# LinXueyuanStdio/LaTeX_OCR

Hardware: AMD Instinct MI355X
Metric: formula-images/sec training step (batch 64, 128x512) (higher is better)
Workload: dtype bf16

## Files before the change

### latex_ocr_amd/csrc/decoder_kernels.hip

```cpp
#include "decoder_kernels.h"
#include "api_util.h"
#include "drop.h"
#include <stdlib.h>

namespace {


LXO_DEV void load4(const float* p, float (&v)[4]) {
    f32x4 a = *reinterpret_cast<const f32x4*>(p);
    v[0] = a[0]; v[1] = a[1]; v[2] = a[2]; v[3] = a[3];
}
LXO_DEV void load4(const bf16_t* p, float (&v)[4]) {
    u32x2 a = *reinterpret_cast<const u32x2*>(p);
    v[0] = __uint_as_float(a[0] << 16); v[1] = __uint_as_float(a[0] & 0xffff0000u);
    v[2] = __uint_as_float(a[1] << 16); v[3] = __uint_as_float(a[1] & 0xffff0000u);
}
LXO_DEV void store4(float* p, const float (&v)[4]) { f32x4 a = {v[0], v[1], v[2], v[3]}; *reinterpret_cast<f32x4*>(p) = a; }
LXO_DEV void store4(bf16_t* p, const float (&v)[4]) { u32x2 a = {pack_bf2(v[0], v[1]), pack_bf2(v[2], v[3])}; *reinterpret_cast<u32x2*>(p) = a; }

LXO_DEV float slab_sum(const Slabs& sl, long long row, int col) {
    float v = 0.f;
    const float* q = sl.p + row * sl.ld + col;
    for (int s = 0; s < sl.n; ++s) v += q[(long long)s * sl.stride];
    return v;
// ... 809 lines not shown
#pragma unroll
            for (int j = 0; j < 4; ++j) rede[wave][k0 + j] = acc[kc][j] * b4[j];
        }
    }
    __syncthreads();
    for (int k = tid; k < E; k += 512) {
        float t = 0.f;
#pragma unroll
        for (int w = 0; w < ATT_W; ++w) t += rede[w][k];
        atomicAdd(&datth[(long long)v * E + k], t);
    }
}

typedef __amdgpu_buffer_rsrc_t ab_rsrc_t;
template <int ATT_U>
LXO_DEV void attb_load(u32x4 (&xi)[ATT_U], u32x2 (&xa)[ATT_U], float (&al)[ATT_U], ab_rsrc_t rim, ab_rsrc_t rai, ab_rsrc_t ral, int base, int n, int lane) {
#pragma unroll
    for (int u = 0; u < ATT_U; ++u) {
        const int r = max(min(base + ATT_W * u, n - 1), 0);
        xi[u] = __builtin_amdgcn_raw_buffer_load_b128(rim, lane * 16, r * 1024, 0);
        xa[u] = __builtin_amdgcn_raw_buffer_load_b64(rai, lane * 8, r * 512, 0);
        al[u] = __uint_as_float(__builtin_amdgcn_raw_buffer_load_b32(ral, 0, r * 4, 0));
    }
}
template <int ATT_U>
LXO_DEV void attb_block(const u32x4 (&xi)[ATT_U], const u32x2 (&xa)[ATT_U], const float (&al)[ATT_U], int base, int n, const float (&dc)[8],
                        const float (&ah)[4], float s, float (&acc)[4], float* de_row, int lane) {
    float pt[ATT_U];
#pragma unroll
    for (int u = 0; u < ATT_U; ++u) {
        float a = 0.f;
#pragma unroll
        for (int e = 0; e < 4; ++e) {
            a = fmaf(__uint_as_float(xi[u][e] << 16), dc[2 * e], a);
            a = fmaf(__uint_as_float(xi[u][e] & 0xffff0000u), dc[2 * e + 1], a);
        }
        pt[u] = a;
    }
#pragma unroll
    for (int o = 32; o > 0; o >>= 1) {
#pragma unroll
        for (int u = 0; u < ATT_U; ++u) pt[u] += __shfl_xor(pt[u], o);
    }
#pragma unroll
    for (int u = 0; u < ATT_U; ++u) {
        const int r = base + ATT_W * u;
        if (r >= n) continue;
        const float d = al[u] * (pt[u] - s);
        if (lane == 0) de_row[r] = d;
        const float x0 = __uint_as_float(xa[u][0] << 16), x1 = __uint_as_float(xa[u][0] & 0xffff0000u);
        const float x2 = __uint_as_float(xa[u][1] << 16), x3 = __uint_as_float(xa[u][1] & 0xffff0000u);
        const float t0 = tanh_ct<bf16_t>(x0 + ah[0]), t1 = tanh_ct<bf16_t>(x1 + ah[1]), t2 = tanh_ct<bf16_t>(x2 + ah[2]), t3 = tanh_ct<bf16_t>(x3 + ah[3]);
        acc[0] = fmaf(d, 1.f - t0 * t0, acc[0]); acc[1] = fmaf(d, 1.f - t1 * t1, acc[1]);
        acc[2] = fmaf(d, 1.f - t2 * t2, acc[2]); acc[3] = fmaf(d, 1.f - t3 * t3, acc[3]);
    }
}
template <int ATT_U>
__global__ __launch_bounds__(512) void attn_bwd_stream_kernel(const bf16_t* __restrict__ att_img, const bf16_t* __restrict__ img,
                                                             const float* __restrict__ att_h, const float* __restrict__ beta,
                                                             const float* __restrict__ alpha, const float* __restrict__ dctx, int lddc,
                                                             const float* __restrict__ ctx, int ldctx,
                                                             float* __restrict__ de, float* __restrict__ datth,
                                                             int R, int Rp, int rows_per, int rev) {
    constexpr int E = 256, C = 512;
    __shared__ float rede[ATT_W][E];
    const int ch = blockIdx.x, v = blockIdx.y;
    const int tid = threadIdx.x, lane = tid & 63, wave = __builtin_amdgcn_readfirstlane(tid >> 6);
    const int r0 = ch * rows_per;
    const int n = min(R, r0 + rows_per) - r0;
    if (n <= 0) return;
    const ab_rsrc_t rim = __builtin_amdgcn_make_buffer_rsrc(const_cast<bf16_t*>(img + ((long long)v * R + r0) * C), 0, n * C * 2, 0x00020000);
    const ab_rsrc_t rai = __builtin_amdgcn_make_buffer_rsrc(const_cast<bf16_t*>(att_img + ((long long)v * R + r0) * E), 0, n * E * 2, 0x00020000);
    const ab_rsrc_t ral = __builtin_amdgcn_make_buffer_rsrc(const_cast<float*>(alpha + (long long)v * Rp + r0), 0, n * 4, 0x00020000);
    const int nblk2 = ((n + ATT_W * ATT_U - 1) / (ATT_W * ATT_U) + 1) & ~1;
#define ABASE(i) (wave + ATT_W * ATT_U * (rev ? nblk2 - 1 - (i) : (i)))
    u32x4 xiA[ATT_U], xiB[ATT_U]; u32x2 xaA[ATT_U], xaB[ATT_U]; float alA[ATT_U], alB[ATT_U];
    attb_load<ATT_U>(xiA, xaA, alA, rim, rai, ral, ABASE(0), n, lane);
    attb_load<ATT_U>(xiB, xaB, alB, rim, rai, ral, ABASE(1), n, lane);
    const int c0 = lane * 8;
    const float* dp = dctx + (long long)v * lddc + c0;
    const float* cp = ctx + (long long)v * ldctx + c0;
    const f32x4 d0 = *reinterpret_cast<const f32x4*>(dp), d1 = *reinterpret_cast<const f32x4*>(dp + 4);
    const f32x4 x0 = *reinterpret_cast<const f32x4*>(cp), x1 = *reinterpret_cast<const f32x4*>(cp + 4);
    const f32x4 a4 = *reinterpret_cast<const f32x4*>(att_h + (long long)v * E + lane * 4);
    const f32x4 b4 = *reinterpret_cast<const f32x4*>(beta + lane * 4);
    float dc[8], ah[4], acc[4] = {0.f, 0.f, 0.f, 0.f};
#pragma unroll
    for (int e = 0; e < 4; ++e) { dc[e] = d0[e]; dc[4 + e] = d1[e]; ah[e] = a4[e]; }
    float s = 0.f;
#pragma unroll
    for (int e = 0; e < 4; ++e) s = fmaf(x0[e], dc[e], fmaf(x1[e], dc[4 + e], s));
    s = wave_sum(s);
    float* de_row = de + (long long)v * Rp + r0;
    for (int it = 0; it + 2 < nblk2; it += 2) {
        attb_block<ATT_U>(xiA, xaA, alA, ABASE(it), n, dc, ah, s, acc, de_row, lane);
        __builtin_amdgcn_sched_barrier(0);
        attb_load<ATT_U>(xiA, xaA, alA, rim, rai, ral, ABASE(it + 2), n, lane);
        __builtin_amdgcn_sched_barrier(0);
        attb_block<ATT_U>(xiB, xaB, alB, ABASE(it + 1), n, dc, ah, s, acc, de_row, lane);
        __builtin_amdgcn_sched_barrier(0);
        attb_load<ATT_U>(xiB, xaB, alB, rim, rai, ral, ABASE(it + 3), n, lane);
        __builtin_amdgcn_sched_barrier(0);
    }
    attb_block<ATT_U>(xiA, xaA, alA, ABASE(nblk2 - 2), n, dc, ah, s, acc, de_row, lane);
    attb_block<ATT_U>(xiB, xaB, alB, ABASE(nblk2 - 1), n, dc, ah, s, acc, de_row, lane);
#undef ABASE
#pragma unroll
    for (int j = 0; j < 4; ++j) rede[wave][lane * 4 + j] = acc[j] * b4[j];
    __syncthreads();
    if (tid < E) {
        float t = 0.f;
#pragma unroll
        for (int w = 0; w < ATT_W; ++w) t += rede[w][tid];
        atomicAdd(&datth[(long long)v * E + tid], t);
    }
}

__global__ __launch_bounds__(256) void att_exp_kernel(const bf16_t* __restrict__ x, bf16_t* __restrict__ out, long long n8) {
    for (long long i = (long long)blockIdx.x * 256 + threadIdx.x; i < n8; i += (long long)gridDim.x * 256) {
        float v[8];
        load8(x + i * 8, v);
#pragma unroll
        for (int e = 0; e < 8; ++e) v[e] = __builtin_amdgcn_exp2f(fminf(fmaxf(v[e] * 2.8853900817779268f, -60.f), 60.f));
        store8(out + i * 8, v);
    }
}

template <typename CT, int KCT>
__global__ __launch_bounds__(256) void datt_img_kernel(const CT* __restrict__ att_img, const float* __restrict__ att_h,
                                                      const float* __restrict__ beta, const float* __restrict__ de,
                                                      CT* __restrict__ dout, float* __restrict__ dbeta, float* __restrict__ dbeta_part,
                                                      int T, int B, int R, int Rp, int E) {
    __shared__ float redb[4][1024];
    const int b = blockIdx.y;
    const int tid = threadIdx.x, lane = tid & 63, wave = tid >> 6;
    const int KC = (E + 255) >> 8;
    float bt[KCT][4], db[KCT][4];
#pragma unroll
    for (int kc = 0; kc < KCT; ++kc) {
        const int k0 = kc * 256 + lane * 4;
#pragma unroll
        for (int j = 0; j < 4; ++j) { bt[kc][j] = (kc < KC && k0 + j < E) ? beta[k0 + j] : 0.f; db[kc][j] = 0.f; }
    }
    const int rbase = blockIdx.x * 16 + wave * 4;
    float x[4][KCT][4], acc[4][KCT][4];
#pragma unroll
    for (int rr = 0; rr < 4; ++rr)
#pragma unroll
        for (int kc = 0; kc < KCT; ++kc) {
            const int k0 = kc * 256 + lane * 4;
#pragma unroll
            for (int j = 0; j < 4; ++j) { x[rr][kc][j] = 0.f; acc[rr][kc][j] = 0.f; }
            if (rbase + rr < R && kc < KC && k0 < E) load4(att_img + ((long long)b * R + rbase + rr) * E + k0, x[rr][kc]);
            if constexpr (is_bf16<CT>::value) {
#pragma unroll
                for (int j = 0; j < 4; ++j) x[rr][kc][j] = __builtin_amdgcn_exp2f(fminf(fmaxf(x[rr][kc][j] * 2.8853900817779268f, -120.f), 120.f));
            }
        }
    float sumd = 0.f;
    if (rbase < R)
    for (int t0 = 0; t0 < T; t0 += 4) {
#pragma unroll
        for (int kc = 0; kc < KCT; ++kc) {
            const int k0 = kc * 256 + lane * 4;
            if (kc < KC && k0 < E) {
                float a[4][4], d[4][4];
#pragma unroll
                for (int tt = 0; tt < 4; ++tt) {
                    const int t = t0 + tt, tc = min(t, T - 1);
                    load4(att_h + ((long long)tc * B + b) * E + k0, a[tt]);
                    f32x4 dq = *reinterpret_cast<const f32x4*>(de + ((long long)tc * B + b) * Rp + rbase);
#pragma unroll
                    for (int rr = 0; rr < 4; ++rr) d[tt][rr] = (t < T && rbase + rr < R) ? dq[rr] : 0.f;
                    if constexpr (is_bf16<CT>::value) {
#pragma unroll
                        for (int j = 0; j < 4; ++j) a[tt][j] = __builtin_amdgcn_exp2f(fminf(fmaxf(a[tt][j] * 2.8853900817779268f, -120.f), 120.f));
                    }
                }
#pragma unroll
                for (int tt = 0; tt < 4; ++tt) {
                    if (d[tt][0] == 0.f && d[tt][1] == 0.f && d[tt][2] == 0.f && d[tt][3] == 0.f) continue;
#pragma unroll
                    for (int rr = 0; rr < 4; ++rr) {
                        const float dd = d[tt][rr];
                        if constexpr (is_bf16<CT>::value) {
                            const f32x2 d4 = {4.f * dd, 4.f * dd}, d2 = {dd, dd}, one = {1.f, 1.f};
                            sumd += dd;
#pragma unroll
                            for (int h = 0; h < 2; ++h) {
                                const f32x2 xs = {x[rr][kc][2 * h], x[rr][kc][2 * h + 1]}, as = {a[tt][2 * h], a[tt][2 * h + 1]};
                                const f32x2 w = __builtin_elementwise_fma(xs, as, one);
                                const f32x2 r = {__builtin_amdgcn_rcpf(w[0]), __builtin_amdgcn_rcpf(w[1])};
                                const f32x2 q = __builtin_elementwise_fma(-r, r, r);
                                f32x2 ac = {acc[rr][kc][2 * h], acc[rr][kc][2 * h + 1]}, dv = {db[kc][2 * h], db[kc][2 * h + 1]};
                                ac = __builtin_elementwise_fma(d4, q, ac);
                                dv = __builtin_elementwise_fma(d2, r, dv);
                                acc[rr][kc][2 * h] = ac[0]; acc[rr][kc][2 * h + 1] = ac[1];
                                db[kc][2 * h] = dv[0]; db[kc][2 * h + 1] = dv[1];
                            }
                        } else {
#pragma unroll
                            for (int j = 0; j < 4; ++j) {
                                const float tau = tanh_ct<CT>(x[rr][kc][j] + a[tt][j]);
                                acc[rr][kc][j] = fmaf(dd, 1.f - tau * tau, acc[rr][kc][j]);
                                db[kc][j] = fmaf(dd, tau, db[kc][j]);
                            }
                        }
                    }
                }
            }
        }
    }
#pragma unroll
    for (int rr = 0; rr < 4; ++rr)
#pragma unroll
        for (int kc = 0; kc < KCT; ++kc) {
            const int k0 = kc * 256 + lane * 4;
            if (rbase + rr < R && kc < KC && k0 < E) {
                float o[4];
#pragma unroll
                for (int j = 0; j < 4; ++j) o[j] = acc[rr][kc][j] * bt[kc][j];
                store4(dout + ((long long)b * R + rbase + rr) * E + k0, o);
            }
        }
#pragma unroll
    for (int kc = 0; kc < KCT; ++kc) {
        const int k0 = kc * 256 + lane * 4;
        if (kc < KC && k0 < E) {
#pragma unroll
            for (int j = 0; j < 4; ++j) redb[wave][k0 + j] = is_bf16<CT>::value ? sumd - 2.f * db[kc][j] : db[kc][j];
        }
    }
    __syncthreads();
    if (dbeta_part) {
        float* slot = dbeta_part + ((long long)blockIdx.y * gridDim.x + blockIdx.x) * E;
        for (int k = tid; k < E; k += 256) slot[k] = redb[0][k] + redb[1][k] + redb[2][k] + redb[3][k];
        return;
    }
    for (int k = tid; k < E; k += 256) atomicAdd(&dbeta[k], redb[0][k] + redb[1][k] + redb[2][k] + redb[3][k]);
}

__global__ __launch_bounds__(256) void add_mean_grad_kernel(float* __restrict__ dimg, const float* __restrict__ dmean, int B, int R, int C) {
    const long long total = (long long)B * R * C;
    const float inv = 1.0f / (float)R;
    for (long long i = (long long)blockIdx.x * 256 + threadIdx.x; i < total; i += (long long)gridDim.x * 256) {
        const int c = (int)(i % C);
        const int b = (int)(i / ((long long)R * C));
        dimg[i] += dmean[(long long)b * C + c] * inv;
    }
}

template <typename CT>
__global__ __launch_bounds__(256) void ce_loss_kernel(const float* __restrict__ logits, const int* __restrict__ formula,
                                                     const int* __restrict__ lengths, CT* __restrict__ dlogits,
                                                     float* __restrict__ loss_acc, float* __restrict__ loss_part, float inv_ntok, const float* __restrict__ ntok_dev,
                                                     const unsigned* __restrict__ chain_err, int B, int T, int V, int Vp) {
    __shared__ float red[8];
    if (chain_err && blockIdx.x == 0 && threadIdx.x == 0 && chain_err[0] != 0u) atomicAdd(&loss_acc[0], __uint_as_float(0x7fc00000u));
    if (ntok_dev) inv_ntok = 1.0f / ntok_dev[0];
    const int lane = threadIdx.x & 63, wave = threadIdx.x >> 6;
    float ce_sum = 0.f, n_sum = 0.f;
    for (int row = blockIdx.x * 4 + wave; row < T * B; row += gridDim.x * 4) {
        const int t = row / B, b = row - t * B;
        const float* lg = logits + (long long)row * Vp;
        CT* dl = dlogits + (long long)row * Vp;
        const bool valid = t < lengths[b];
        int tgt = formula[(long long)b * T + t];
        tgt = tgt < 0 ? 0 : (tgt >= V ? V - 1 : tgt);
        float m = -3.0e38f;
        for (int j = lane; j < V; j += 64) m = fmaxf(m, lg[j]);
        m = wave_max(m);
        float l = 0.f;
        for (int j = lane; j < V; j += 64) l += expf(lg[j] - m);
        l = wave_sum(l);
        const float lse = m + logf(l);
        const float scale = valid ? inv_ntok : 0.f;
        for (int j = lane; j < Vp; j += 64) {
            float g = 0.f;
            if (j < V) g = (expf(lg[j] - lse) - (j == tgt ? 1.f : 0.f)) * scale;
            dl[j] = from_f32<CT>(g);
        }
        if (valid) { ce_sum += lse - lg[tgt]; n_sum += 1.0f; }
    }
    if (lane == 0) { red[wave] = ce_sum; red[4 + wave] = n_sum; }
    __syncthreads();
    if (threadIdx.x == 0) {
        const float c = red[0] + red[1] + red[2] + red[3], n = red[4] + red[5] + red[6] + red[7];
        if (loss_part) { loss_part[2 * blockIdx.x] = c; loss_part[2 * blockIdx.x + 1] = n; }
        else if (n > 0.f) { atomicAdd(&loss_acc[0], c); atomicAdd(&loss_acc[1], n); }
    }
}

template <typename CT, int KV>
__global__ __launch_bounds__(256) void ce_loss_rows_kernel(const float* __restrict__ logits, const int* __restrict__ formula,
                                                          const int* __restrict__ lengths, CT* __restrict__ dlogits,
                                                          float* __restrict__ loss_acc, float* __restrict__ loss_part, float inv_ntok, const float* __restrict__ ntok_dev,
                                                          const unsigned* __restrict__ chain_err, int B, int T, int V, int Vp) {
    __shared__ float red[8];
    if (chain_err && blockIdx.x == 0 && threadIdx.x == 0 && chain_err[0] != 0u) atomicAdd(&loss_acc[0], __uint_as_float(0x7fc00000u));
    if (ntok_dev) inv_ntok = 1.0f / ntok_dev[0];
    const int lane = threadIdx.x & 63, wave = threadIdx.x >> 6;
    float ce_sum = 0.f, n_sum = 0.f;
    for (int row = blockIdx.x * 4 + wave; row < T * B; row += gridDim.x * 4) {
        const int t = row / B, b = row - t * B;
        const float* lg = logits + (long long)row * Vp;
        CT* dl = dlogits + (long long)row * Vp;
        const bool valid = t < lengths[b];
        int tgt = formula[(long long)b * T + t];
        tgt = tgt < 0 ? 0 : (tgt >= V ? V - 1 : tgt);
        const float xt = lg[tgt];
        float x[KV];
#pragma unroll
        for (int q = 0; q < KV / 4; ++q) {
            const int j0 = 4 * (lane + 64 * q);
            const f32x4 v = *reinterpret_cast<const f32x4*>(lg + (j0 < Vp ? j0 : 0));
#pragma unroll
            for (int e = 0; e < 4; ++e) x[4 * q + e] = (j0 + e < V) ? v[e] : -3.0e38f;
        }
        float m = x[0];
#pragma unroll
        for (int e = 1; e < KV; ++e) m = fmaxf(m, x[e]);
        m = wave_max(m);
        float l = 0.f;
#pragma unroll
        for (int e = 0; e < KV; ++e) l += is_bf16<CT>::value ? __expf(x[e] - m) : expf(x[e] - m);
        l = wave_sum(l);
        const float lse = m + logf(l);
        const float scale = valid ? inv_ntok : 0.f;
#pragma unroll
        for (int q = 0; q < KV / 4; ++q) {
            const int j0 = 4 * (lane + 64 * q);
            if (j0 >= Vp) continue;
            float g[4];
#pragma unroll
            for (int e = 0; e < 4; ++e) {
                const int j = j0 + e;
                const float pr = is_bf16<CT>::value ? __expf(x[4 * q + e] - lse) : expf(x[4 * q + e] - lse);
                g[e] = j < V ? (pr - (j == tgt ? 1.f : 0.f)) * scale : 0.f;
            }
            if constexpr (is_bf16<CT>::value) { const u32x2 pk = {pack_bf2(g[0], g[1]), pack_bf2(g[2], g[3])}; *reinterpret_cast<u32x2*>(dl + j0) = pk; }
            else { const f32x4 gv = {g[0], g[1], g[2], g[3]}; *reinterpret_cast<f32x4*>(dl + j0) = gv; }
        }
        if (valid) { ce_sum += lse - xt; n_sum += 1.0f; }
    }
    if (lane == 0) { red[wave] = ce_sum; red[4 + wave] = n_sum; }
    __syncthreads();
    if (threadIdx.x == 0) {
        const float c = red[0] + red[1] + red[2] + red[3], n = red[4] + red[5] + red[6] + red[7];
        if (loss_part) { loss_part[2 * blockIdx.x] = c; loss_part[2 * blockIdx.x + 1] = n; }
        else if (n > 0.f) { atomicAdd(&loss_acc[0], c); atomicAdd(&loss_acc[1], n); }
    }
}

__global__ __launch_bounds__(256) void colsum_kernel(const float* __restrict__ a, int lda, float* __restrict__ out, int M, int N, int rows_per_block) {
    const int n = blockIdx.x * 256 + threadIdx.x;
    const int m0 = blockIdx.y * rows_per_block, m1 = min(M, m0 + rows_per_block);
    if (n >= N) return;
    float s = 0.f;
    for (int m = m0; m < m1; ++m) s += a[(long long)m * lda + n];
    atomicAdd(&out[n], s);
}

__global__ __launch_bounds__(256) void colsum4_kernel(const float* __restrict__ a, int lda, float* __restrict__ out, int M, int N, int rows_per_block) {
    __shared__ f32x4 red[4][64];
    const int cq = threadIdx.x & 63, ry = threadIdx.x >> 6;
    const int n = (blockIdx.x * 64 + cq) * 4;
    const int m0 = blockIdx.y * rows_per_block, m1 = min(M, m0 + rows_per_block);
    const int nl = n < N ? n : 0;
    f32x4 s = {0.f, 0.f, 0.f, 0.f};
    for (int mb = m0 + ry; mb < m1; mb += 32) {
        f32x4 v[8];
#pragma unroll
        for (int u = 0; u < 8; ++u) { const int m = min(mb + 4 * u, m1 - 1); v[u] = *reinterpret_cast<const f32x4*>(a + (long long)m * lda + nl); }
#pragma unroll
        for (int u = 0; u < 8; ++u) if (mb + 4 * u < m1) s += v[u];
    }
    red[ry][cq] = s;
    __syncthreads();
    if (ry == 0 && n < N) {
        const f32x4 t = red[0][cq] + red[1][cq] + red[2][cq] + red[3][cq];
#pragma unroll
        for (int e = 0; e < 4; ++e) atomicAdd(&out[n + e], t[e]);
    }
}


template <typename AT>
__global__ __launch_bounds__(256) void colsum_part_kernel(const AT* __restrict__ a, long long lda, float* __restrict__ part, long long M, int N, int rows_per) {
    const int n = blockIdx.x * 256 + threadIdx.x;
    const long long m0 = (long long)blockIdx.y * rows_per, m1 = m0 + rows_per < M ? m0 + rows_per : M;
    if (n >= N) return;
    float s = 0.f;
// ... 722 lines not shown
    if (C % 64) return -2;
    if (dt == LXO_BF16) LAUNCH((rowmean_kernel<bf16_t>), dim3(C / 64, B), (const bf16_t*)img, mean, R, C);
    else LAUNCH((rowmean_kernel<float>), dim3(C / 64, B), (const float*)img, mean, R, C);
    DONE;
}
int lxo_k_embed_gather(int dt, const float* table, const float* start, const int* formula, void* out, int B, int T, int D, int Dp, int V, hipStream_t st) {
    const int g = grid1((long long)T * B * Dp);
    if (dt == LXO_BF16) LAUNCH((embed_gather_kernel<bf16_t>), g, table, start, formula, (bf16_t*)out, B, T, D, Dp, V);
    else LAUNCH((embed_gather_kernel<float>), g, table, start, formula, (float*)out, B, T, D, Dp, V);
    DONE;
}
int lxo_k_embed_rows(int dt, const float* table, const float* start, const int* ids, void* out, int n, int D, int Dp, int V, hipStream_t st) {
    const int g = grid1((long long)n * Dp);
    if (dt == LXO_BF16) LAUNCH((embed_rows_kernel<bf16_t>), g, table, start, ids, (bf16_t*)out, n, D, Dp, V);
    else LAUNCH((embed_rows_kernel<float>), g, table, start, ids, (float*)out, n, D, Dp, V);
    DONE;
}
int lxo_k_embed_table(int dt, const float* table, const float* start, void* out, int V, int D, int Dp, hipStream_t st) {
    const int g = grid1((long long)(V + 1) * Dp);
    if (dt == LXO_BF16) LAUNCH((embed_table_kernel<bf16_t>), g, table, start, (bf16_t*)out, V, D, Dp);
    else LAUNCH((embed_table_kernel<float>), g, table, start, (float*)out, V, D, Dp);
    DONE;
}
int lxo_k_lstm_fwd(const float* z, Slabs zs, const float* c_prev, float* gates, float* c_out, float* h_out, float* ht_out, int ldh, Drop dr, int B, int U, hipStream_t st) {
    LAUNCH(lstm_fwd_kernel, grid1((long long)B * U), z, zs, c_prev, gates, c_out, h_out, ht_out, ldh, dr, B, U);
    DONE;
}
int lxo_k_lstm_bwd(const float* gates, const float* c_prev, const float* c_cur, Slabs s1, Slabs s3, Slabs s4, int off4,
                   float* dcc, float* dz, Drop dr, int carry_rows, int B, int U, hipStream_t st) {
    LAUNCH(lstm_bwd_kernel, grid1((long long)B * U), gates, c_prev, c_cur, s1, s3, s4, off4, dcc, dz, dr, carry_rows, B, U);
    DONE;
}
int lxo_k_tanh_bwd(const float* a, int lda, Slabs carry, const float* o, int ldo, float* g, int ldg, void* gb, int ldgb, Drop dr, int carry_rows, int rows, int cols, hipStream_t st) {
    LAUNCH(tanh_bwd_kernel, grid1((long long)rows * cols / 4), a, lda, carry, o, ldo, g, ldg, (bf16_t*)gb, ldgb, dr, carry_rows, rows, cols);
    DONE;
}
__global__ __launch_bounds__(256) static void slab_reduce_kernel(Slabs sl, float* __restrict__ o, int ldo, int rows, int cols) {
    const int total = rows * (cols >> 2);
    for (int i = blockIdx.x * 256 + threadIdx.x; i < total; i += gridDim.x * 256) {
        const int r = i / (cols >> 2), c = (i - r * (cols >> 2)) << 2;
        *reinterpret_cast<f32x4*>(o + (long long)r * ldo + c) = slab_sum4(sl, r, c);
    }
}
int lxo_k_slab_reduce(Slabs sl, float* o, int ldo, int rows, int cols, hipStream_t st) {
    LAUNCH(slab_reduce_kernel, grid1((long long)rows * cols / 4), sl, o, ldo, rows, cols);
    DONE;
}
int lxo_k_tanh_finalize(Slabs sl, float* o, int ldo, Drop dr, int rows, int cols, hipStream_t st) {
    LAUNCH(tanh_finalize_kernel, grid1((long long)rows * cols / 4), sl, o, ldo, dr, rows, cols);
    DONE;
}
static int att_u(int rows_per) {
    static int forced = -1;
    if (forced < 0) { const char* e = getenv("LXO_ATT_U"); forced = e ? atoi(e) : 0; }
    if (forced == 7 || forced == 8) return forced;
    return (rows_per + 55) / 56 <= (rows_per + 63) / 64 ? 7 : 8;
}
int lxo_k_attn_fwd(int dt, const void* att_img, const void* img, const float* att_h, Slabs ahs, float* att_h_out, const float* beta, float* alpha, float* part,
                   float* ctx, int ldctx, void* ctxb, int ldcb, int nv, int R, int Rp, int E, int C, int beam, int nch, int rev, hipStream_t st, const void* att_exp) {
    if (E > 1024 || C > 512 || nch < 1 || nch > 32) return -2;
    const int rows_per = cdiv(R, nch);
    dim3 grid(nch, nv);
    static int split = -1;
    if (split < 0) { const char* e = getenv("LXO_ATT_SPLIT"); split = (e && e[0] == '1') ? 1 : 0; }
    const int epl = dt == LXO_BF16 ? 8 : 4;
    if (split && ahs.n == 0 && att_h && R <= 1024 && C % 64 == 0 && E % epl == 0 && E <= 64 * epl && ((E / epl) & (E / epl - 1)) == 0) {
        if (dt == LXO_BF16) {
            hipLaunchKernelGGL((attn_scores_kernel<bf16_t, 8>), grid, dim3(512), 0, st, (const bf16_t*)att_img, att_h, beta, part, R, Rp, E, beam, rows_per);
            hipLaunchKernelGGL((attn_ctx_kernel<bf16_t, 8>), dim3(C / 64, nv), dim3(512), 0, st, (const bf16_t*)img, part, alpha, ctx, ldctx, (bf16_t*)ctxb, ldcb, R, Rp, C, beam);
        } else {
            hipLaunchKernelGGL((attn_scores_kernel<float, 8>), grid, dim3(512), 0, st, (const float*)att_img, att_h, beta, part, R, Rp, E, beam, rows_per);
            hipLaunchKernelGGL((attn_ctx_kernel<float, 8>), dim3(C / 64, nv), dim3(512), 0, st, (const float*)img, part, alpha, ctx, ldctx, (bf16_t*)ctxb, ldcb, R, Rp, C, beam);
        }
        DONE;
    }
    static int beam_shared = -1;
    if (beam_shared < 0) { const char* e = getenv("LXO_ATT_BEAM_SHARED"); beam_shared = (e && e[0] == '0') ? 0 : 1; }
    if (beam_shared && (beam == 2 || beam == 3 || beam == 5 || (beam == 1 && att_exp && dt == LXO_BF16)) && ahs.n == 0 && att_h && E <= 256 && C <= 512 && nv % beam == 0) {
        const int nimg = nv / beam;
        int nb = cdiv(512, nimg);
        if (nb > 16) nb = 16;
        const int by_rows = R / 32 > 0 ? R / 32 : 1;
        if (nb > by_rows) nb = by_rows;
        const int need = cdiv(R, 1024);
        if (nb < need) nb = need;
        const int rpb = cdiv(R, nb);
        const dim3 gb(nb, nimg);
#define ABM(CT_, U_, NB_, X_, OCC_, AI_) hipLaunchKernelGGL((attn_fwd_part_beam_kernel<CT_, U_, NB_, X_, OCC_>), gb, dim3(512), 0, st, (const CT_*)(AI_), (const CT_*)img, att_h, beta, alpha, part, R, Rp, E, C, nb, rpb, rev)
        if (dt == LXO_BF16 && att_exp) { if (beam == 1) ABM(bf16_t, 4, 1, true, 4, att_exp); else if (beam == 2) ABM(bf16_t, 4, 2, true, 4, att_exp); else if (beam == 3) ABM(bf16_t, 4, 3, true, 4, att_exp); else ABM(bf16_t, 2, 5, true, 4, att_exp); }
        else if (dt == LXO_BF16) { if (beam == 2) ABM(bf16_t, 4, 2, false, 2, att_img); else if (beam == 3) ABM(bf16_t, 4, 3, false, 2, att_img); else ABM(bf16_t, 4, 5, false, 2, att_img); }
        else { if (beam == 2) ABM(float, 4, 2, false, 2, att_img); else if (beam == 3) ABM(float, 4, 3, false, 2, att_img); else ABM(float, 4, 5, false, 2, att_img); }
#undef ABM
        hipLaunchKernelGGL(attn_fwd_combine_kernel, dim3(4, nv), dim3(256), 0, st, part, alpha, ctx, ldctx, (bf16_t*)ctxb, ldcb, R, Rp, C, nb, rpb);
        DONE;
    }
#define AF_ARGS att_h, ahs, att_h_out, beta, alpha, part, R, Rp, E, C, beam, nch, rows_per, rev
    if (dt == LXO_BF16) {
        if (E <= 256) { if (att_u(rows_per) == 8) hipLaunchKernelGGL((attn_fwd_part_kernel<bf16_t, 1, 8>), grid, dim3(512), 0, st, (const bf16_t*)att_img, (const bf16_t*)img, AF_ARGS); else hipLaunchKernelGGL((attn_fwd_part_kernel<bf16_t, 1, 7>), grid, dim3(512), 0, st, (const bf16_t*)att_img, (const bf16_t*)img, AF_ARGS); }
        else { if (att_u(rows_per) == 8) hipLaunchKernelGGL((attn_fwd_part_kernel<bf16_t, 4, 8>), grid, dim3(512), 0, st, (const bf16_t*)att_img, (const bf16_t*)img, AF_ARGS); else hipLaunchKernelGGL((attn_fwd_part_kernel<bf16_t, 4, 7>), grid, dim3(512), 0, st, (const bf16_t*)att_img, (const bf16_t*)img, AF_ARGS); }
    } else {
        if (E <= 256) { if (att_u(rows_per) == 8) hipLaunchKernelGGL((attn_fwd_part_kernel<float, 1, 8>), grid, dim3(512), 0, st, (const float*)att_img, (const float*)img, AF_ARGS); else hipLaunchKernelGGL((attn_fwd_part_kernel<float, 1, 7>), grid, dim3(512), 0, st, (const float*)att_img, (const float*)img, AF_ARGS); }
        else { if (att_u(rows_per) == 8) hipLaunchKernelGGL((attn_fwd_part_kernel<float, 4, 8>), grid, dim3(512), 0, st, (const float*)att_img, (const float*)img, AF_ARGS); else hipLaunchKernelGGL((attn_fwd_part_kernel<float, 4, 7>), grid, dim3(512), 0, st, (const float*)att_img, (const float*)img, AF_ARGS); }
    }
#undef AF_ARGS
    hipLaunchKernelGGL(attn_fwd_combine_kernel, dim3(4, nv), dim3(256), 0, st, part, alpha, ctx, ldctx, (bf16_t*)ctxb, ldcb, R, Rp, C, nch, rows_per);
    DONE;
}
int lxo_k_att_exp(const void* att_img, void* att_exp, long long n, hipStream_t st) {
    if (n % 8) return -2;
    LAUNCH(att_exp_kernel, grid1(n / 8, 256, 4096), (const bf16_t*)att_img, (bf16_t*)att_exp, n / 8);
    DONE;
}
int lxo_k_attn_bwd(int dt, const void* att_img, const void* att_exp, const void* img, const float* att_h, const float* beta, const float* alpha,
                   Slabs dcs, int dcoff, float* dctx_out, int lddc, const float* ctx, int ldctx, float* de, float* datth,
                   int nv, int R, int Rp, int E, int C, int nch, int rev, hipStream_t st) {
    if (E > 1024 || C > 512 || nch < 1 || nch > 32) return -2;
    const int rows_per = cdiv(R, nch);
    dim3 grid(nch, nv);
    static int stream2 = -1;
    if (stream2 < 0) { const char* e = getenv("LXO_ATT_BWD2"); stream2 = (e && e[0] == '1') ? 1 : 0; }
    if (stream2 && dt == LXO_BF16 && E == 256 && C == 512 && dcs.n == 1 && lddc % 4 == 0 && ldctx % 4 == 0 && (long long)rows_per * 1024 < (1LL << 31)) {
        const float* dctx = dcs.p + dcoff;
        if (dctx_out) return -2;
        hipLaunchKernelGGL((attn_bwd_stream_kernel<4>), grid, dim3(512), 0, st, (const bf16_t*)att_img, (const bf16_t*)img, att_h, beta, alpha, dctx, dcs.ld,
                           ctx, ldctx, de, datth, R, Rp, rows_per, rev);
        DONE;
    }
#define AB_ARGS att_h, beta, alpha, dcs, dcoff, dctx_out, lddc, ctx, ldctx, de, datth, R, Rp, E, C, rows_per, rev
    if (dt == LXO_BF16 && att_exp && E <= 256) {
        if (att_u(rows_per) == 8) hipLaunchKernelGGL((attn_bwd_part_kernel<bf16_t, 1, 8, true>), grid, dim3(512), 0, st, (const bf16_t*)att_exp, (const bf16_t*)img, AB_ARGS);
        else hipLaunchKernelGGL((attn_bwd_part_kernel<bf16_t, 1, 7, true>), grid, dim3(512), 0, st, (const bf16_t*)att_exp, (const bf16_t*)img, AB_ARGS);
    } else if (dt == LXO_BF16) {
        if (E <= 256) { if (att_u(rows_per) == 8) hipLaunchKernelGGL((attn_bwd_part_kernel<bf16_t, 1, 8>), grid, dim3(512), 0, st, (const bf16_t*)att_img, (const bf16_t*)img, AB_ARGS); else hipLaunchKernelGGL((attn_bwd_part_kernel<bf16_t, 1, 7>), grid, dim3(512), 0, st, (const bf16_t*)att_img, (const bf16_t*)img, AB_ARGS); }
        else { if (att_u(rows_per) == 8) hipLaunchKernelGGL((attn_bwd_part_kernel<bf16_t, 4, 8>), grid, dim3(512), 0, st, (const bf16_t*)att_img, (const bf16_t*)img, AB_ARGS); else hipLaunchKernelGGL((attn_bwd_part_kernel<bf16_t, 4, 7>), grid, dim3(512), 0, st, (const bf16_t*)att_img, (const bf16_t*)img, AB_ARGS); }
    } else {
        if (E <= 256) { if (att_u(rows_per) == 8) hipLaunchKernelGGL((attn_bwd_part_kernel<float, 1, 8>), grid, dim3(512), 0, st, (const float*)att_img, (const float*)img, AB_ARGS); else hipLaunchKernelGGL((attn_bwd_part_kernel<float, 1, 7>), grid, dim3(512), 0, st, (const float*)att_img, (const float*)img, AB_ARGS); }
        else { if (att_u(rows_per) == 8) hipLaunchKernelGGL((attn_bwd_part_kernel<float, 4, 8>), grid, dim3(512), 0, st, (const float*)att_img, (const float*)img, AB_ARGS); else hipLaunchKernelGGL((attn_bwd_part_kernel<float, 4, 7>), grid, dim3(512), 0, st, (const float*)att_img, (const float*)img, AB_ARGS); }
    }
#undef AB_ARGS
    DONE;
}
int lxo_k_det_reduce(const float* part, int nslot, long long stride, int N, float* out, hipStream_t st) {
    if (nslot <= 0 || N <= 0) return 0;
    hipLaunchKernelGGL(det_reduce_kernel, dim3(cdiv(N, 16)), dim3(256), 0, st, part, nslot, stride, N, out);
    DONE;
}
int lxo_k_datt_img(int dt, const void* att_img, const float* att_h, const float* beta, const float* de, void* dout, float* dbeta,
                   int T, int B, int R, int Rp, int E, DetScratch det, hipStream_t st) {
    dim3 grid(cdiv(R, 16), B);
    if (E > 1024) return -2;
    float* part = nullptr;
    if (det.p) { if ((size_t)grid.x * grid.y * E > det.floats) return -6; part = det.p; }
    if (dt == LXO_BF16) {
        if (E <= 256) hipLaunchKernelGGL((datt_img_kernel<bf16_t, 1>), grid, dim3(256), 0, st, (const bf16_t*)att_img, att_h, beta, de, (bf16_t*)dout, dbeta, part, T, B, R, Rp, E);
        else hipLaunchKernelGGL((datt_img_kernel<bf16_t, 4>), grid, dim3(256), 0, st, (const bf16_t*)att_img, att_h, beta, de, (bf16_t*)dout, dbeta, part, T, B, R, Rp, E);
    } else {
        if (E <= 256) hipLaunchKernelGGL((datt_img_kernel<float, 1>), grid, dim3(256), 0, st, (const float*)att_img, att_h, beta, de, (float*)dout, dbeta, part, T, B, R, Rp, E);
        else hipLaunchKernelGGL((datt_img_kernel<float, 4>), grid, dim3(256), 0, st, (const float*)att_img, att_h, beta, de, (float*)dout, dbeta, part, T, B, R, Rp, E);
    }
    if (part) return lxo_k_det_reduce(part, (int)(grid.x * grid.y), E, E, dbeta, st);
    DONE;
}
int lxo_k_add_mean_grad(float* dimg, const float* dmean, int B, int R, int C, hipStream_t st) {
    LAUNCH(add_mean_grad_kernel, grid1((long long)B * R * C), dimg, dmean, B, R, C);
    DONE;
}
int lxo_k_ce_loss(int dt, const float* logits, const int* formula, const int* lengths, void* dlogits, float* loss_acc, float inv_ntok,
                  const float* ntok_dev, const unsigned* chain_err, int B, int T, int V, int Vp, DetScratch det, hipStream_t st) {
    int g = cdiv(T * B, 4);
    float* part = (det.p && det.floats >= 1024) ? det.p : nullptr;
    if (Vp % 4 == 0 && Vp <= 1024 && (((uintptr_t)logits | (uintptr_t)dlogits) & 15) == 0) {
        if (g > (part ? 512 : 2048)) g = part ? 512 : 2048;
#define CE_ROWS(CT_, KV_) LAUNCH((ce_loss_rows_kernel<CT_, KV_>), g, logits, formula, lengths, (CT_*)dlogits, loss_acc, part, inv_ntok, ntok_dev, chain_err, B, T, V, Vp)
        if (dt == LXO_BF16) { if (Vp <= 256) CE_ROWS(bf16_t, 4); else if (Vp <= 512) CE_ROWS(bf16_t, 8); else CE_ROWS(bf16_t, 16); }
        else { if (Vp <= 256) CE_ROWS(float, 4); else if (Vp <= 512) CE_ROWS(float, 8); else CE_ROWS(float, 16); }
#undef CE_ROWS
        if (part) return lxo_k_det_reduce(part, g, 2, 2, loss_acc, st);
        DONE;
    }
    if (g > 512) g = 512;
    if (dt == LXO_BF16) LAUNCH((ce_loss_kernel<bf16_t>), g, logits, formula, lengths, (bf16_t*)dlogits, loss_acc, part, inv_ntok, ntok_dev, chain_err, B, T, V, Vp);
    else LAUNCH((ce_loss_kernel<float>), g, logits, formula, lengths, (float*)dlogits, loss_acc, part, inv_ntok, ntok_dev, chain_err, B, T, V, Vp);
    if (part) return lxo_k_det_reduce(part, g, 2, 2, loss_acc, st);
    DONE;
}
int lxo_k_score(int dt, const float* logits, const int* formula, const int* lengths, float* logp_out, int* top1_out, float* seq_out,
                const unsigned* chain_err, int B, int T, int V, int Vp, hipStream_t st) {
    int g = cdiv(T * B, 4);
    if (Vp % 4 == 0 && Vp <= 1024 && ((uintptr_t)logits & 15) == 0) {
        if (g > 2048) g = 2048;
#define SC_ROWS(BF_, KV_) LAUNCH((score_rows_kernel<BF_, KV_>), g, logits, formula, lengths, logp_out, top1_out, chain_err, B, T, V, Vp)
        if (dt == LXO_BF16) { if (Vp <= 256) SC_ROWS(true, 4); else if (Vp <= 512) SC_ROWS(true, 8); else SC_ROWS(true, 16); }
        else { if (Vp <= 256) SC_ROWS(false, 4); else if (Vp <= 512) SC_ROWS(false, 8); else SC_ROWS(false, 16); }
#undef SC_ROWS
    } else {
        LAUNCH(score_kernel, g > 512 ? 512 : g, logits, formula, lengths, logp_out, top1_out, chain_err, B, T, V, Vp);
    }
    if (seq_out) LAUNCH(score_seq_kernel, cdiv(B, 256), logp_out, lengths, seq_out, chain_err, B, T);
    DONE;
}
int lxo_k_colsum_det(const void* a, int bf16, long long lda, float* out, long long M, int N, DetScratch det, hipStream_t st) {
    if (!det.p) return -6;
    if (M <= 0 || N <= 0) return 0;
    long long maxslots = (long long)(det.floats / (size_t)N);
    if (maxslots < 1) return -6;
    if (maxslots > 1024) maxslots = 1024;
    long long rows_per = (M + maxslots - 1) / maxslots;
    if (rows_per < 64) rows_per = 64;
    const int nrb = (int)((M + rows_per - 1) / rows_per);
    if (bf16) hipLaunchKernelGGL((colsum_part_kernel<bf16_t>), dim3(cdiv(N, 256), nrb), dim3(256), 0, st, (const bf16_t*)a, lda, det.p, M, N, (int)rows_per);
    else hipLaunchKernelGGL((colsum_part_kernel<float>), dim3(cdiv(N, 256), nrb), dim3(256), 0, st, (const float*)a, lda, det.p, M, N, (int)rows_per);
    return lxo_k_det_reduce(det.p, nrb, N, N, out, st);
}
int lxo_k_colsum(const float* a, long long lda, float* out, long long M, int N, DetScratch det, hipStream_t st) {
    if (det.p) return lxo_k_colsum_det(a, 0, lda, out, M, N, det, st);
    const int rpb = 64;
    if (N % 4 == 0 && lda % 4 == 0 && ((uintptr_t)a & 15) == 0 && M > 0)
        hipLaunchKernelGGL(colsum4_kernel, dim3(cdiv(N, 256), cdiv((int)M, rpb)), dim3(256), 0, st, a, (int)lda, out, (int)M, N, rpb);
    else
    hipLaunchKernelGGL(colsum_kernel, dim3(cdiv(N, 256), cdiv((int)M, rpb)), dim3(256), 0, st, a, (int)lda, out, (int)M, N, rpb);
    DONE;
}
int lxo_k_embed_scatter(const float* demb, const int* formula, float* dtable, float* dstart, int B, int T, int D, int V, int det, hipStream_t st) {
    if (D <= 256) { hipLaunchKernelGGL(embed_scatter_rows_kernel, dim3(V + 1, det ? 1 : 16), dim3(256), 0, st, demb, formula, dtable, dstart, B, T, D, V, det); DONE; }
    if (det) return -2;
    LAUNCH(embed_scatter_kernel, grid1((long long)T * B * D), demb, formula, dtable, dstart, B, T, D, V);
    DONE;
}
int lxo_k_init_bwd(const float* dcc, Slabs dxh, const float* c0, const float* rec0, int ldr, float* dpre, int B, int U, int O, hipStream_t st) {
    LAUNCH(init_bwd_kernel, grid1((long long)B * (2 * U + O)), dcc, dxh, c0, rec0, ldr, dpre, B, U, O);
    DONE;
}
#define DEC_VARIANT(KERNEL, grid, block, ...)                                                                         \
    do {                                                                                                               \
        if (prefix && allow) hipLaunchKernelGGL((KERNEL<true, true>), dim3(grid), dim3(block), 0, st, __VA_ARGS__);    \
        else if (prefix) hipLaunchKernelGGL((KERNEL<true, false>), dim3(grid), dim3(block), 0, st, __VA_ARGS__);       \
        else if (allow) hipLaunchKernelGGL((KERNEL<false, true>), dim3(grid), dim3(block), 0, st, __VA_ARGS__);        \
        else hipLaunchKernelGGL((KERNEL<false, false>), dim3(grid), dim3(block), 0, st, __VA_ARGS__);                  \
    } while (0)
int lxo_k_argmax(const float* logits, int Vp, int V, int n, int id_end, int* ids_step, int* ids_out, int max_steps, int step,
                 int* finished, int* n_unfinished, hipStream_t st, float* logp_out, const DecPrefix* prefix, const DecAllow* allow) {
    const DecPrefix pf = prefix ? *prefix : DecPrefix{};
    const DecAllow al = allow ? *allow : DecAllow{};
    DEC_VARIANT(argmax_kernel, cdiv(n, 4), 256, logits, Vp, V, n, id_end, ids_step, ids_out, max_steps, step, finished, n_unfinished, logp_out, pf, al);
    DONE;
}
int lxo_k_beam_step(float* logits, int Vp, int V, int nimg, int k, int id_end, int time, float div_gamma, float div_prob, int div_seed,
                    float* scratch, float* logp, int* finished,
                    int* ids_step, int* parents_step, int* ids_out, int* par_out, int max_steps, int* n_unfinished, hipStream_t st,
                    float* scores_out, const DecPrefix* prefix, const DecAllow* allow) {
    if (k > 16 || k > V) return -2;
    DivPen dp = {0.f, 0u, (unsigned)div_seed, scratch};
    if (div_gamma > 0.f && div_gamma != 1.f && div_prob > 0.f) {
        dp.log_gamma = logf(div_gamma);
        dp.thr = div_prob >= 1.f ? 16777216u : (unsigned)(div_prob * 16777216.0f);
    }
    static int fast = -1;
    if (fast < 0) { const char* e = getenv("LXO_BEAM_FAST"); fast = (e && e[0] == '0') ? 0 : 1; }
    const DecPrefix pf = prefix ? *prefix : DecPrefix{};
    const DecAllow al = allow ? *allow : DecAllow{};
    if (fast && dp.log_gamma == 0.f && (long long)k * V <= BS_TH * BS_NPT && k * BS_NW <= 64) {
        DEC_VARIANT(beam_step_fast_kernel, nimg, BS_TH, logits, Vp, V, k, id_end, time, logp, finished, ids_step, parents_step, ids_out, par_out, max_steps, n_unfinished, scores_out, pf, al);
    } else
        DEC_VARIANT(beam_step_kernel, nimg, 256, logits, Vp, V, k, id_end, time, dp, logp, finished, ids_step, parents_step, ids_out, par_out, max_steps, n_unfinished, scores_out, pf, al);
    DONE;
}
int lxo_k_beam_gather(float* rec, int ldr, int XH, float* cs, int U, const int* parents, int k, float* tmp_rec, float* tmp_cs, int n, void* recb, int ldrb, hipStream_t st) {
    if (k >= 1 && k <= BP_KMAX && n % k == 0) {
        LAUNCH(beam_permute_kernel, dim3(n / k, cdiv(XH + U, 256)), rec, ldr, XH, cs, U, parents, k, (bf16_t*)recb, ldrb);
        DONE;
    }
    LAUNCH(beam_gather_kernel, grid1((long long)n * (XH + U)), rec, ldr, XH, cs, U, parents, k, tmp_rec, tmp_cs, n);
    LAUNCH(beam_scatter_kernel, grid1((long long)n * (XH + U)), rec, ldr, XH, cs, U, tmp_rec, tmp_cs, n, (bf16_t*)recb, ldrb);
    DONE;
}
int lxo_k_tile_rows(const float* src, int lds, float* dst, int ldd, int n, int k, int cols, hipStream_t st) {
    LAUNCH(tile_rows_kernel, grid1((long long)n * cols), src, lds, dst, ldd, n, k, cols);
    DONE;
}
int lxo_k_global_norm_scale(long long n, const float* g, float clip, float* sumsq_tmp, float* out, hipStream_t st) {
    const int nparts = grid1(n, 256 * 8, 1024);
    LAUNCH(sumsq_kernel, nparts, g, n, sumsq_tmp);
    hipLaunchKernelGGL(clip_scale_kernel, dim3(1), dim3(1), 0, st, sumsq_tmp, nparts, clip, out);
    DONE;
}
int lxo_k_simple_opt(float* p, const float* g, float* slot, long long n, float lr, int mode, const float* scale, hipStream_t st) {
    if (mode < 1 || mode > 3 || (mode > 1 && !slot)) return -2;
    LAUNCH(simple_opt_kernel, grid1(n, 256 * 4, 4096), p, g, slot, n, lr, mode, scale);
    DONE;
}
int lxo_k_chain_guard(const unsigned* err_fwd, const unsigned* err_bwd, const float* probe, float* scale, int have_scale, unsigned* status, hipStream_t st) {
    hipLaunchKernelGGL(chain_guard_kernel, dim3(1), dim3(1), 0, st, err_fwd, err_bwd, probe, scale, have_scale, status);
    DONE;
}
int lxo_k_chain_poison(const unsigned* err_fwd, const unsigned* err_bwd, float* probe, hipStream_t st) {
    hipLaunchKernelGGL(chain_poison_kernel, dim3(1), dim3(1), 0, st, err_fwd, err_bwd, probe);
    DONE;
}
int lxo_k_adam(float* p, const float* g, float* m, float* v, long long n, float lr_t, float b1, float b2, float eps, const float* scale, hipStream_t st) {
    LAUNCH(adam_kernel, grid1(n, 256 * 4, 4096), p, g, m, v, n, lr_t, b1, b2, eps, scale);
    DONE;
}
```

Measured before the change: 8666.

## Stage exp of att_h through double-buffered LDS in bf16 attention backward

Adds a bf16-specific datt_img kernel. Each time chunk of att_h is exponentiated once per block and written to a double-buffered shared-memory tile, instead of every wave reloading and re-exponentiating it. The next chunk's global loads are prefetched while the current one is computed, and larger time steps are used for small E. The cost is more LDS use and a barrier per chunk. The float path stays on the generic kernel with the bf16 branch removed.

Result: no change. 8649 (-0.2%).

```diff
diff --git a/latex_ocr_amd/csrc/decoder_kernels.hip b/latex_ocr_amd/csrc/decoder_kernels.hip
--- a/latex_ocr_amd/csrc/decoder_kernels.hip
+++ b/latex_ocr_amd/csrc/decoder_kernels.hip
@@ -985,12 +985,7 @@
 #pragma unroll
             for (int j = 0; j < 4; ++j) { x[rr][kc][j] = 0.f; acc[rr][kc][j] = 0.f; }
             if (rbase + rr < R && kc < KC && k0 < E) load4(att_img + ((long long)b * R + rbase + rr) * E + k0, x[rr][kc]);
-            if constexpr (is_bf16<CT>::value) {
-#pragma unroll
-                for (int j = 0; j < 4; ++j) x[rr][kc][j] = __builtin_amdgcn_exp2f(fminf(fmaxf(x[rr][kc][j] * 2.8853900817779268f, -120.f), 120.f));
-            }
-        }
-    float sumd = 0.f;
+        }
     if (rbase < R)
     for (int t0 = 0; t0 < T; t0 += 4) {
 #pragma unroll
@@ -1005,72 +1000,186 @@
                     f32x4 dq = *reinterpret_cast<const f32x4*>(de + ((long long)tc * B + b) * Rp + rbase);
 #pragma unroll
                     for (int rr = 0; rr < 4; ++rr) d[tt][rr] = (t < T && rbase + rr < R) ? dq[rr] : 0.f;
-                    if constexpr (is_bf16<CT>::value) {
-#pragma unroll
-                        for (int j = 0; j < 4; ++j) a[tt][j] = __builtin_amdgcn_exp2f(fminf(fmaxf(a[tt][j] * 2.8853900817779268f, -120.f), 120.f));
+                }
+#pragma unroll
+                for (int tt = 0; tt < 4; ++tt) {
+                    if (d[tt][0] == 0.f && d[tt][1] == 0.f && d[tt][2] == 0.f && d[tt][3] == 0.f) continue;
+#pragma unroll
+                    for (int rr = 0; rr < 4; ++rr) {
+                        const float dd = d[tt][rr];
+#pragma unroll
+                        for (int j = 0; j < 4; ++j) {
+                            const float tau = tanh_ct<CT>(x[rr][kc][j] + a[tt][j]);
+                            acc[rr][kc][j] = fmaf(dd, 1.f - tau * tau, acc[rr][kc][j]);
+                            db[kc][j] = fmaf(dd, tau, db[kc][j]);
+                        }
                     }
                 }
-#pragma unroll
-                for (int tt = 0; tt < 4; ++tt) {
-                    if (d[tt][0] == 0.f && d[tt][1] == 0.f && d[tt][2] == 0.f && d[tt][3] == 0.f) continue;
-#pragma unroll
-                    for (int rr = 0; rr < 4; ++rr) {
-                        const float dd = d[tt][rr];
-                        if constexpr (is_bf16<CT>::value) {
-                            const f32x2 d4 = {4.f * dd, 4.f * dd}, d2 = {dd, dd}, one = {1.f, 1.f};
-                            sumd += dd;
-#pragma unroll
-                            for (int h = 0; h < 2; ++h) {
-                                const f32x2 xs = {x[rr][kc][2 * h], x[rr][kc][2 * h + 1]}, as = {a[tt][2 * h], a[tt][2 * h + 1]};
-                                const f32x2 w = __builtin_elementwise_fma(xs, as, one);
-                                const f32x2 r = {__builtin_amdgcn_rcpf(w[0]), __builtin_amdgcn_rcpf(w[1])};
-                                const f32x2 q = __builtin_elementwise_fma(-r, r, r);
-                                f32x2 ac = {acc[rr][kc][2 * h], acc[rr][kc][2 * h + 1]}, dv = {db[kc][2 * h], db[kc][2 * h + 1]};
-                                ac = __builtin_elementwise_fma(d4, q, ac);
-                                dv = __builtin_elementwise_fma(d2, r, dv);
-                                acc[rr][kc][2 * h] = ac[0]; acc[rr][kc][2 * h + 1] = ac[1];
-                                db[kc][2 * h] = dv[0]; db[kc][2 * h + 1] = dv[1];
-                            }
-                        } else {
+            }
+        }
+    }
+#pragma unroll
+    for (int rr = 0; rr < 4; ++rr)
+#pragma unroll
+        for (int kc = 0; kc < KCT; ++kc) {
+            const int k0 = kc * 256 + lane * 4;
+            if (rbase + rr < R && kc < KC && k0 < E) {
+                float o[4];
+#pragma unroll
+                for (int j = 0; j < 4; ++j) o[j] = acc[rr][kc][j] * bt[kc][j];
+                store4(dout + ((long long)b * R + rbase + rr) * E + k0, o);
+            }
+        }
+#pragma unroll
+    for (int kc = 0; kc < KCT; ++kc) {
+        const int k0 = kc * 256 + lane * 4;
+        if (kc < KC && k0 < E) {
+#pragma unroll
+            for (int j = 0; j < 4; ++j) redb[wave][k0 + j] = db[kc][j];
+        }
+    }
+    __syncthreads();
+    if (dbeta_part) {
+        float* slot = dbeta_part + ((long long)blockIdx.y * gridDim.x + blockIdx.x) * E;
+        for (int k = tid; k < E; k += 256) slot[k] = redb[0][k] + redb[1][k] + redb[2][k] + redb[3][k];
+        return;
+    }
+    for (int k = tid; k < E; k += 256) atomicAdd(&dbeta[k], redb[0][k] + redb[1][k] + redb[2][k] + redb[3][k]);
+}
+
+template <int KCT>
+__global__ __launch_bounds__(256) void datt_img_kernel(const bf16_t* __restrict__ att_img, const float* __restrict__ att_h,
+                                                      const float* __restrict__ beta, const float* __restrict__ de,
+                                                      bf16_t* __restrict__ dout, float* __restrict__ dbeta, float* __restrict__ dbeta_part,
+                                                      int T, int B, int R, int Rp, int E) {
+    constexpr int TS = KCT == 1 ? 8 : 4;
+    constexpr int NCH = TS * KCT / 4;
+    __shared__ float ea[2 * TS * KCT * 256];
+    const int b = blockIdx.y;
+    const int tid = threadIdx.x, lane = tid & 63, wave = __builtin_amdgcn_readfirstlane(tid >> 6);
+    const int KC = (E + 255) >> 8;
+    const int rbase = blockIdx.x * 16 + wave * 4;
+    const bool live = rbase < R;
+    float x[4][KCT][4], acc[4][KCT][4], db[KCT][4];
+#pragma unroll
+    for (int kc = 0; kc < KCT; ++kc) {
+        const int k0 = kc * 256 + lane * 4;
+#pragma unroll
+        for (int j = 0; j < 4; ++j) db[kc][j] = 0.f;
+#pragma unroll
+        for (int rr = 0; rr < 4; ++rr) {
+#pragma unroll
+            for (int j = 0; j < 4; ++j) { x[rr][kc][j] = 0.f; acc[rr][kc][j] = 0.f; }
+            if (rbase + rr < R && kc < KC && k0 < E) load4(att_img + ((long long)b * R + rbase + rr) * E + k0, x[rr][kc]);
+#pragma unroll
+            for (int j = 0; j < 4; ++j) x[rr][kc][j] = __builtin_amdgcn_exp2f(fminf(fmaxf(x[rr][kc][j] * 2.8853900817779268f, -120.f), 120.f));
+        }
+    }
+    float sa[NCH][4];
+    auto stage_load = [&](int t0) {
+#pragma unroll
+        for (int c = 0; c < NCH; ++c) {
+            const int ch = c * 4 + wave, tc = min(t0 + ch / KCT, T - 1), k0 = min((ch % KCT) * 256 + lane * 4, E - 4);
+            load4(att_h + ((long long)tc * B + b) * E + k0, sa[c]);
+        }
+    };
+    auto stage_store = [&](int buf) {
+#pragma unroll
+        for (int c = 0; c < NCH; ++c) {
+            const int ch = c * 4 + wave;
+            f32x4 v;
+#pragma unroll
+            for (int j = 0; j < 4; ++j) v[j] = __builtin_amdgcn_exp2f(fminf(fmaxf(sa[c][j] * 2.8853900817779268f, -120.f), 120.f));
+            *reinterpret_cast<f32x4*>(&ea[(buf * TS * KCT + ch) * 256 + lane * 4]) = v;
+        }
+    };
+    f32x4 d[TS];
+    unsigned rm[4];
+#pragma unroll
+    for (int rr = 0; rr < 4; ++rr) rm[rr] = rbase + rr < R ? 0xffffffffu : 0u;
+    const float* de_w = de + (long long)b * Rp + rbase;
+    const long long de_step = (long long)B * Rp;
+    auto load_d = [&](int t0) {
+#pragma unroll
+        for (int tt = 0; tt < TS; ++tt) d[tt] = *reinterpret_cast<const f32x4*>(de_w + min(t0 + tt, T - 1) * de_step);
+    };
+    auto read_a = [&](f32x4 (&a)[KCT], int buf, int tt) {
+#pragma unroll
+        for (int kc = 0; kc < KCT; ++kc)
+            if (KCT == 1 || kc < KC) a[kc] = *reinterpret_cast<const f32x4*>(&ea[((buf * TS + tt) * KCT + kc) * 256 + lane * 4]);
+    };
+    float sumd = 0.f;
+    stage_load(0);
+    if (live) load_d(0);
+    stage_store(0);
+    __syncthreads();
+    for (int t0 = 0, buf = 0; t0 < T; t0 += TS, buf ^= 1) {
+        stage_load(t0 + TS);
+        if (live) {
+            f32x4 an[KCT];
+            read_a(an, buf, 0);
+#pragma unroll
+            for (int tt = 0; tt < TS; ++tt) {
+                f32x4 a[KCT];
+#pragma unroll
+                for (int kc = 0; kc < KCT; ++kc) a[kc] = an[kc];
+                if (tt + 1 < TS) read_a(an, buf, tt + 1);
+                float dm[4];
+#pragma unroll
+                for (int rr = 0; rr < 4; ++rr) dm[rr] = __uint_as_float(__float_as_uint(d[tt][rr]) & rm[rr]);
+                if (t0 + tt >= T || ((__float_as_uint(dm[0]) | __float_as_uint(dm[1]) | __float_as_uint(dm[2]) | __float_as_uint(dm[3])) << 1) == 0u) continue;
+#pragma unroll
+                for (int rr = 0; rr < 4; ++rr) sumd += dm[rr];
+#pragma unroll
+                for (int kc = 0; kc < KCT; ++kc) {
+                    if (KCT == 1 || kc < KC) {
+#pragma unroll
+                        for (int rr = 0; rr < 4; ++rr) {
+                            const float dd = dm[rr];
 #pragma unroll
                             for (int j = 0; j < 4; ++j) {
-                                const float tau = tanh_ct<CT>(x[rr][kc][j] + a[tt][j]);
-                                acc[rr][kc][j] = fmaf(dd, 1.f - tau * tau, acc[rr][kc][j]);
-                                db[kc][j] = fmaf(dd, tau, db[kc][j]);
+                                const float w = fmaf(x[rr][kc][j], a[kc][j], 1.f);
+                                const float r = __builtin_amdgcn_rcpf(w);
+                                const float q = fmaf(-r, r, r);
+                                acc[rr][kc][j] = fmaf(dd, q, acc[rr][kc][j]);
+                                db[kc][j] = fmaf(dd, r, db[kc][j]);
                             }
                         }
                     }
                 }
             }
-        }
-    }
-#pragma unroll
-    for (int rr = 0; rr < 4; ++rr)
-#pragma unroll
-        for (int kc = 0; kc < KCT; ++kc) {
-            const int k0 = kc * 256 + lane * 4;
-            if (rbase + rr < R && kc < KC && k0 < E) {
-                float o[4];
-#pragma unroll
-                for (int j = 0; j < 4; ++j) o[j] = acc[rr][kc][j] * bt[kc][j];
-                store4(dout + ((long long)b * R + rbase + rr) * E + k0, o);
-            }
-        }
+            load_d(t0 + TS);
+        }
+        stage_store(buf ^ 1);
+        __syncthreads();
+    }
 #pragma unroll
     for (int kc = 0; kc < KCT; ++kc) {
         const int k0 = kc * 256 + lane * 4;
         if (kc < KC && k0 < E) {
-#pragma unroll
-            for (int j = 0; j < 4; ++j) redb[wave][k0 + j] = is_bf16<CT>::value ? sumd - 2.f * db[kc][j] : db[kc][j];
+            float bt4[4];
+#pragma unroll
+            for (int j = 0; j < 4; ++j) bt4[j] = 4.f * beta[k0 + j];
+#pragma unroll
+            for (int rr = 0; rr < 4; ++rr)
+                if (rbase + rr < R) {
+                    float o[4];
+#pragma unroll
+                    for (int j = 0; j < 4; ++j) o[j] = acc[rr][kc][j] * bt4[j];
+                    store4(dout + ((long long)b * R + rbase + rr) * E + k0, o);
+                }
+#pragma unroll
+            for (int j = 0; j < 4; ++j) ea[wave * 1024 + k0 + j] = sumd - 2.f * db[kc][j];
         }
     }
     __syncthreads();
+    const float* redb = ea;
     if (dbeta_part) {
         float* slot = dbeta_part + ((long long)blockIdx.y * gridDim.x + blockIdx.x) * E;
-        for (int k = tid; k < E; k += 256) slot[k] = redb[0][k] + redb[1][k] + redb[2][k] + redb[3][k];
+        for (int k = tid; k < E; k += 256) slot[k] = redb[k] + redb[1024 + k] + redb[2048 + k] + redb[3072 + k];
         return;
     }
-    for (int k = tid; k < E; k += 256) atomicAdd(&dbeta[k], redb[0][k] + redb[1][k] + redb[2][k] + redb[3][k]);
+    for (int k = tid; k < E; k += 256) atomicAdd(&dbeta[k], redb[k] + redb[1024 + k] + redb[2048 + k] + redb[3072 + k]);
 }
 
 __global__ __launch_bounds__(256) void add_mean_grad_kernel(float* __restrict__ dimg, const float* __restrict__ dmean, int B, int R, int C) {
@@ -2099,8 +2208,8 @@
     float* part = nullptr;
     if (det.p) { if ((size_t)grid.x * grid.y * E > det.floats) return -6; part = det.p; }
     if (dt == LXO_BF16) {
-        if (E <= 256) hipLaunchKernelGGL((datt_img_kernel<bf16_t, 1>), grid, dim3(256), 0, st, (const bf16_t*)att_img, att_h, beta, de, (bf16_t*)dout, dbeta, part, T, B, R, Rp, E);
-        else hipLaunchKernelGGL((datt_img_kernel<bf16_t, 4>), grid, dim3(256), 0, st, (const bf16_t*)att_img, att_h, beta, de, (bf16_t*)dout, dbeta, part, T, B, R, Rp, E);
+        if (E <= 256) hipLaunchKernelGGL((datt_img_kernel<1>), grid, dim3(256), 0, st, (const bf16_t*)att_img, att_h, beta, de, (bf16_t*)dout, dbeta, part, T, B, R, Rp, E);
+        else hipLaunchKernelGGL((datt_img_kernel<4>), grid, dim3(256), 0, st, (const bf16_t*)att_img, att_h, beta, de, (bf16_t*)dout, dbeta, part, T, B, R, Rp, E);
     } else {
         if (E <= 256) hipLaunchKernelGGL((datt_img_kernel<float, 1>), grid, dim3(256), 0, st, (const float*)att_img, att_h, beta, de, (float*)dout, dbeta, part, T, B, R, Rp, E);
         else hipLaunchKernelGGL((datt_img_kernel<float, 4>), grid, dim3(256), 0, st, (const float*)att_img, att_h, beta, de, (float*)dout, dbeta, part, T, B, R, Rp, E);
```
